# EmanueleCosenza/polyphemus

Hardware: AMD Instinct MI355X
Metric: bar-graphs/sec VAE fwd+bwd (+loss +Adam), LMD2 4-track x 32-ts synthetic (higher is better)
Workload: dtype f32 (fp16-pair MFMA products)

## Files before the change

include/polyphemus_hip.h:

```cpp
#ifndef POLYPHEMUS_HIP_H
#define POLYPHEMUS_HIP_H

#include <stdint.h>

#ifdef __cplusplus
extern "C" {
#endif

typedef void* pm_stream_t;

enum {
  PM_OK = 0,
  PM_E_INVALID = -1,
  PM_E_LAUNCH = -2,
  PM_E_UNSUPPORTED = -3
};

enum { PM_N_REL = 6, PM_N_DIST = 32, PM_N_SLOTS = 15, PM_N_PITCH = 131, PM_N_DUR = 99, PM_N_TOK = 230 };

#define PM_ABI_VERSION 9
int pm_abi_version(void);
const char* pm_build_info(void);

int pm_set_deterministic(int32_t on);
// ... 152 lines not shown
                               const float* bias , int32_t use_classes, float* h ,
                               double* col_stats , pm_stream_t stream);
int pm_gcl_forward_from_planes_h2(const uint16_t* a_planes, int64_t plane_stride, const int32_t* plan, int32_t N, int32_t E,
                                  int32_t G, int32_t d, const uint16_t* w_frag, const float* bias, int32_t use_classes,
                                  float* h, double* col_stats, const float* a_scale, float w_scale, pm_stream_t stream);
int pm_rows_times_weight(const float* X, int32_t ldx, int32_t N, int32_t K, const uint16_t* w_frag, int32_t kind,
                         int32_t w_tiles, int32_t Nout, const float* bias , float* C, int32_t ldc,
                         pm_stream_t stream);
int pm_rows_times_weight_longk(const float* X, int32_t ldx, int32_t N, int32_t K, const uint16_t* w_frag, int32_t kind,
                               int32_t w_pitch, int32_t Nout, float* C, int32_t ldc, pm_stream_t stream);
int pm_rows_tn_weight_grad(const float* A, int32_t lda, int32_t M, const float* B, int32_t ldb, int32_t Nn, int32_t K,
                           float* C , int32_t ldc, float* colsum_a , pm_stream_t stream);
typedef struct PmNormSums {
  const float* h;
  const float* mean; const float* var; const float* gamma; const float* beta;
  float eps; int32_t relu;
  double* acc3;
  uint32_t* absmax_out;
} PmNormSums;
int pm_segreduce_bwd_norm(const float* x, const float* T, const float* dA, const float* dres, const int32_t* plan,
                          int32_t N, int32_t E, int32_t G, int32_t d, float dropout_p, uint32_t seed,
                          uint32_t layer_uid, int32_t compact, float* dx, float* dT, const PmNormSums* next_norm,
                          pm_stream_t stream);
int pm_segreduce_bwd(const float* x, const float* T, const float* dA ,
                     const float* dres ,
                     const int32_t* plan, int32_t N, int32_t E, int32_t G, int32_t d, float dropout_p,
                     uint32_t seed, uint32_t layer_uid, int32_t compact, float* dx ,
                     float* dT , pm_stream_t stream);

int pm_bar_aggregate_fwd(const float* x, const float* T, const int32_t* plan, int32_t N, int32_t E, int32_t G, int32_t d,
                         float dropout_p, uint32_t seed, uint32_t layer_uid, uint16_t* planes, int64_t plane_stride,
                         const PmH2* h2 , pm_stream_t stream);
int pm_bar_aggregate_bwd(const float* x, const float* T, const float* dA , const float* dres ,
                         const int32_t* plan, int32_t N, int32_t E, int32_t G, int32_t d, float dropout_p, uint32_t seed,
                         uint32_t layer_uid, float* dx , float* dT ,
                         const PmNormSums* next_norm , pm_stream_t stream);

enum { PM_GEMM_RELU = 1, PM_GEMM_ACCUM = 2,
       PM_GEMM_RELU_ADD = 16 ,
       PM_GEMM_ZEROED = 8 ,
       PM_GEMM_PARTITION = 4  };
int pm_gemm_config(int32_t transA, int32_t M, int32_t N, int32_t K);
int pm_gemm_force_config(int32_t cfg);
int pm_gemm_f32(int transA, int transB, int32_t M, int32_t N, int32_t K, const float* A, int32_t lda,
                const float* B, int32_t ldb, float* C, int32_t ldc, const float* bias, int flags,
                int split_k, const int32_t* rowmap, int32_t rows_per_entry, const int32_t* dyn_entries,
// ... 110 lines not shown
int pm_embed_gather(const float* tables, const int32_t* tokens , const uint8_t* is_drum,
                    int32_t N, int32_t d, int32_t n_slots, float* X , pm_stream_t stream);
int pm_embed_bwd_scatter(const float* dX , const int32_t* tokens, const int32_t* plan, int32_t N,
                         int32_t E, int32_t G, int32_t d, int32_t n_slots,
                         float* S , pm_stream_t stream);
int pm_chord_pad_fwd(const float* tables, const float* chord_w , const float* chord_b,
                     const uint8_t* is_drum, int32_t N, int32_t d, int32_t n_slots, float* cvec ,
                     float* y , pm_stream_t stream);
int pm_chord_pad_bwd(const float* dy , const uint8_t* is_drum, int32_t N, int32_t d, int32_t n_slots,
                     const float* tables, const float* chord_w, float* gsum ,
                     float* d_chord_w , float* S , pm_stream_t stream);
int pm_chord_pad_vec(const float* tables, const float* chord_w, const float* chord_b, int32_t d, int32_t n_slots,
                     float* cvec , pm_stream_t stream);
int pm_chord_tables_fwd(const float* tables , const float* chord_w , int32_t d, int32_t n_slots,
                        float* PT, const float* chord_b , float* cvec ,
                        pm_stream_t stream);
int pm_chord_sum_fwd(const float* PT, const float* cvec, const int32_t* tokens , const uint8_t* is_drum, int32_t N,
                     int32_t d, int32_t n_slots, float* x0 , pm_stream_t stream);
int pm_chord_sum_bwd(const float* dy , const int32_t* tokens, const int32_t* plan, int32_t N, int32_t E, int32_t G,
                     int32_t d , int32_t n_slots, float* Gt, pm_stream_t stream);
int pm_chord_tables_bwd_w(const float* Gt, const float* tables, int32_t d, int32_t n_slots, float* d_chord_w ,
                          float* d_chord_b , pm_stream_t stream);
int pm_chord_tables_bwd_x(const float* Gt, const float* chord_w, int32_t d, int32_t n_slots, float* S , pm_stream_t stream);
int pm_embed_tables_bwd(const float* S, const float* w_pitch_drum, const float* b_pitch_drum,
                        const float* w_pitch_nd, const float* b_pitch_nd, const float* w_dur, const float* b_dur,
                        const float* bn_drum_g, const float* bn_nd_g, const float* bn_dur_g, const float* stats,
                        const int32_t* tok_hist, int32_t d, float eps, float* dw_pitch_drum, float* db_pitch_drum,
                        float* dw_pitch_nd, float* db_pitch_nd, float* dw_dur, float* db_dur, float* dg_drum,
                        float* dbeta_drum, float* dg_nd, float* dbeta_nd, float* dg_dur, float* dbeta_dur,
                        pm_stream_t stream);

int pm_embed_tables_bwd_sync(const float* S, const float* w_pitch_drum, const float* b_pitch_drum, const float* w_pitch_nd,
                             const float* b_pitch_nd, const float* w_dur, const float* b_dur, const float* bn_drum_g,
                             const float* bn_nd_g, const float* bn_dur_g, const float* stats, const int32_t* tok_hist,
                             int32_t d, float eps, float* dw_pitch_drum, float* db_pitch_drum, float* dw_pitch_nd,
                             float* db_pitch_nd, float* dw_dur, float* db_dur, float* dg_drum, float* dbeta_drum,
                             float* dg_nd, float* dbeta_nd, float* dg_dur, float* dbeta_dur, double* sums_out,
                             const double* sums_global, const int32_t* hist_global, pm_stream_t stream);

int pm_gate_fwd(const float* x , const float* w , const float* b , int32_t N,
                int32_t d, float* g , pm_stream_t stream);
int pm_attnpool_fwd(const float* x, const float* g, const float* g_mean, const float* g_var, float eps,
                    const float* bn_g, const float* bn_b, const int32_t* plan, int32_t N, int32_t E, int32_t G,
                    int32_t d, float* alpha , float* out , pm_stream_t stream);
int pm_attnpool_bwd(const float* x, const float* g, const float* g_mean, const float* g_var, float eps,
                    const float* bn_g, const float* alpha, const float* dout , const float* gate_w,
// ... 240 lines not shown
```

polyphemus_amd/_lib.py:

```python
from __future__ import annotations

import ctypes as C
import os
from typing import Optional

import torch

_HERE = os.path.dirname(os.path.abspath(__file__))
LIB_PATH = os.environ.get("PM_LIB_PATH") or os.path.join(_HERE, "libpolyphemus_hip.so")

PROF_NCLASS = 40
PLAN_FIELDS = ["rowptr", "csr_src", "csr_dist", "csr_eid", "colptr", "csc_dst", "csc_reldist", "csc_eid",
               "csc_invcnt", "node_bar", "bar_ptr", "group_list", "group_cnt", "tok_hist", "row_list", "node_trel", "trk_list", "trk_cnt", "scratch"]

_SIGS = {
    "pm_plan_layout": "iiip",
    "pm_gcl_tile_order": "piipi",
    "pm_row_tile_order": "ipi",
    "pm_plan_build": "pppppppiiiiips",
    "pm_edge_attrs_to_ids": "pipps",
    "pm_tokens_from_onehot": "pips",
    "pm_batch_flags": "pppiipps",
    "pm_edge_table": "ppips",
    "pm_edge_table_bwd": "pipps",
    "pm_graph_count": "pippppps",
    "pm_graph_emit": "piippllppppppps",
    "pm_binary_from_logits": "pifpps",
    "pm_mtp_from_logits": "ppilppps",
    "pm_segreduce_fwd": "pppiiiifuuips",
    "pm_segreduce_fwd_planes": "pppiiiifuuipls",
    "pm_gcl_forward_fused": "pppiiiifuuppipppls",
    "pm_gcl_input_grad_fused": "plpiiiipips",
    "pm_gcl_input_grad_bn": "pplpiiiipips",
    "pm_chord_pad_vec": "pppiips",
    "pm_chord_tables_fwd": "ppiippps",
    "pm_chord_sum_fwd": "ppppiiips",
    "pm_chord_sum_bwd": "pppiiiiips",
    "pm_chord_tables_bwd_w": "ppiipps",
    "pm_chord_tables_bwd_x": "ppiips",
    "pm_bn_bwd_sums": "ppiippfppips",
    "pm_gcl_weight_grad_fused": "plplpiiiiips",
    "pm_gcl_forward_from_planes": "plpiiiippipps",
    "pm_rows_times_weight": "piiipiiippis",
    "pm_rows_times_weight_longk": "piiipiiipis",
    "pm_rows_tn_weight_grad": "piipiiipips",
    "pm_segreduce_bwd": "pppppiiiifuuipps",
    "pm_segreduce_bwd_norm": "pppppiiiifuuippps",
    "pm_gemm_f32": "iiiiipipipipiipips",
    "pm_gemm_f32_grouped": "iiiiipipipipiipipilllliis",
    "pm_gemm_f32_desc": "ps",
    "pm_gemm_config": "iiii",
    "pm_gemm_force_config": "i",
    "pm_bn_stats": "piiippppfps",
    "pm_bn_small_fwd": "piifpppipppppfs",
    "pm_bn_small_bwd": "ppiippfppipppps",
    "pm_bn_apply": "piiippfpppips",
    "pm_bn_partial_sums": "ppiiippfppipps",
    "pm_bn_stats_from_sums": "pDippppfs",
    "pm_bn_bwd_from_sums": "ppiiippfppippDppppps",
    "pm_bn_bwd": "ppiiippfppippppps",
    "pm_bn_apply_fused": "piipfpppipppppfs",
    "pm_bn_bwd_fused": "ppiippfppipppppplis",
    "pm_split_planes": "plpls",
    "pm_split_planes_frag": "piiiillps",
    "pm_relu_bwd": "pplps",
    "pm_add": "pplps",
    "pm_bn_counters_update": "ppppis",
    "pm_grad_accumulate": "pplfis",
    "pm_colsum_acc": "piiips",
    "pm_colsum_rows_acc": "piipipips",
# ... 226 lines not shown
```

polyphemus_amd/csrc/chord.hip:

```cpp
#include "common.h"
#include <stdlib.h>

#define EMB_V PM_N_PITCH

namespace {
__host__ __device__ inline int64_t pt_off(int g, int s, int kind, int S, int d) {
  return (((int64_t)g * S + s) * 2 + kind) * EMB_V * d;
}

template <bool AK, bool BK, int KC, class FA, class FB, class FC>
__device__ inline void small_product(int M, int Nn, int K, int m0, int n0, FA a_at, FB b_at, FC c_out) {
  constexpr int PA = 34, PB = 68;
  constexpr int NA = KC / 8, NB = KC / 4;
  static_assert(KC % 8 == 0, "32 x KC and 64 x KC values over 256 threads");
  __shared__ __attribute__((aligned(16))) float sA[KC * PA], sB[KC * PB];
  const int t = threadIdx.x, tm = t >> 4, tn = t & 15;
  float acc[2][4] = {{0.f, 0.f, 0.f, 0.f}, {0.f, 0.f, 0.f, 0.f}};
  float ra[NA], rb[NB];
  auto request = [&](int k0) {
#pragma unroll
    for (int i = 0; i < NA; ++i) {
      const int idx = t + i * 256;
      const int m = AK ? idx / KC : idx & 31, k = AK ? idx % KC : idx >> 5;
      ra[i] = (m0 + m < M && k0 + k < K) ? a_at(m0 + m, k0 + k) : 0.f;
    }
#pragma unroll
    for (int i = 0; i < NB; ++i) {
      const int idx = t + i * 256;
      const int n = BK ? idx / KC : idx & 63, k = BK ? idx % KC : idx >> 6;
      rb[i] = (n0 + n < Nn && k0 + k < K) ? b_at(n0 + n, k0 + k) : 0.f;
    }
  };
  request(0);
  for (int k0 = 0; k0 < K; k0 += KC) {
#pragma unroll
    for (int i = 0; i < NA; ++i) {
      const int idx = t + i * 256;
      const int m = AK ? idx / KC : idx & 31, k = AK ? idx % KC : idx >> 5;
// ... 38 lines not shown
      const float* td = tables + ((int64_t)(2 + g) * EMB_V + 98) * dh;
      float a0 = 0.f, a1 = 0.f, a2 = 0.f, a3 = 0.f;
      const int i0 = S * d + lane, i1 = PM_N_SLOTS * d;
      int i = i0;
      for (; i + 192 < i1; i += 256) {
        const int c0 = i % d, c1 = (i + 64) % d, c2 = (i + 128) % d, c3 = (i + 192) % d;
        a0 += (c0 < dh ? tp[c0] : td[c0 - dh]) * wrow[i];
        a1 += (c1 < dh ? tp[c1] : td[c1 - dh]) * wrow[i + 64];
        a2 += (c2 < dh ? tp[c2] : td[c2 - dh]) * wrow[i + 128];
        a3 += (c3 < dh ? tp[c3] : td[c3 - dh]) * wrow[i + 192];
      }
      for (; i < i1; i += 64) { const int c0 = i % d; a0 += (c0 < dh ? tp[c0] : td[c0 - dh]) * wrow[i]; }
      const float acc = pm_wave_sum((a0 + a1) + (a2 + a3));
      if (lane == 0) cvec[g * d + o] = acc + bc[o];
    }
    return;
  }
  const int mt = blockIdx.x / ntn, nt = blockIdx.x % ntn, s = blockIdx.y, kind = blockIdx.z >> 1, g = blockIdx.z & 1;
  const int V = kind == 0 ? PM_N_PITCH : PM_N_DUR;
  if (mt * 32 >= V) return;
  const float* T = tables + (int64_t)(kind * 2 + g) * EMB_V * dh;
  const float* W = Wc + (int64_t)s * d + kind * dh;
  float* out = PT + pt_off(g, s, kind, S, d);
  small_product<true, true, 64>(V, d, dh, mt * 32, nt * 64,
                            [&](int v, int c) { return T[(int64_t)v * dh + c]; },
                            [&](int j, int c) { return W[(int64_t)j * PM_N_SLOTS * d + c]; },
                            [&](int v, int j, float x) { out[(int64_t)v * d + j] = x; });
}
extern "C" int pm_chord_tables_fwd(const float* tables, const float* Wc, int32_t d, int32_t n_slots, float* PT, const float* bc,
                                   float* cvec, pm_stream_t stream) {
  if (!tables || !Wc || !PT || d <= 0 || (d & 7) || n_slots < 1 || n_slots > PM_N_SLOTS || (cvec && !bc)) return PM_E_INVALID;
  const int ntm = (int)pm_cdiv(EMB_V, 32), ntn = (int)pm_cdiv(d, 64);
  hipLaunchKernelGGL(k_chord_tables_fwd, dim3(ntm * ntn, n_slots, cvec ? 5 : 4), dim3(256), 0, (hipStream_t)stream, tables, Wc, d,
                     n_slots, PT, bc, cvec);
  return pm_check_launch();
}

template <int SMAX>
__global__ void __launch_bounds__(256) k_chord_sum_fwd(const float* __restrict__ PT, const float* __restrict__ cvec,
                                                       const int* __restrict__ tok, const uint8_t* __restrict__ is_drum, int N,
                                                       int d, int S, float* __restrict__ x0, unsigned* __restrict__ absmax) {
  const int n = blockIdx.x * 4 + (threadIdx.x >> 6), lane = threadIdx.x & 63;
  __shared__ unsigned s_amax;
  if (threadIdx.x == 0) s_amax = 0u;
  float amax = 0.f;
  if (n < N) {
  const int g = is_drum[n] ? 0 : 1;
// ... 208 lines not shown
    Gv[(int64_t)pad * d + j] = all - oth;
  }
}
extern "C" int pm_chord_sum_bwd(const float* dY, const int32_t* tokens, const int32_t* plan, int32_t N, int32_t E, int32_t G_,
                                int32_t d, int32_t n_slots, float* Gt, pm_stream_t stream) {
  if (!dY || !tokens || !plan || !Gt || N <= 0 || d <= 0 || (d % 32) || d > 512 || n_slots < 1 || n_slots > PM_N_SLOTS ||
      (int64_t)N * d * 4 >= 0x7fffffffLL)
    return PM_E_INVALID;
  hipStream_t st = (hipStream_t)stream;
  PmPlanView pv = pm_plan_view(plan, N, E, G_);
  constexpr int chunk_env = 0;
  const int per = chunk_env > 0 ? chunk_env : 640;
  constexpr bool skip_pad = true;
  const int nb = (int)pm_cdiv(N, per) + 1;
  const int waves = d / 32 > 8 ? 8 : d / 32, cblks = (d / 32 + waves - 1) / waves;
  if (d / 32 != waves * cblks) return PM_E_INVALID;
  hipLaunchKernelGGL(k_chord_sum_bwd, dim3(nb, n_slots, 2 * cblks), dim3(64 * waves), 0, st, dY, tokens, pv.group_list, pv.group_cnt,
                     N, d, n_slots, per, skip_pad ? 1 : 0, Gt, pm_det_gate(st));
  if (skip_pad && 2 * n_slots > 1)
    hipLaunchKernelGGL(k_chord_pad_fix, dim3((unsigned)pm_cdiv(d, 64), 2 * n_slots, 2), dim3(256), 0, st, Gt, d, n_slots);
  return pm_check_launch();
}

__global__ void __launch_bounds__(256) k_chord_tables_bwd_w(const float* __restrict__ G, const float* __restrict__ tables, int d,
                                                            int S, float* __restrict__ dWc, float* __restrict__ db, unsigned* gate) {
  const int dh = d / 2, ntn = (dh + 63) / 64;
  const int mt = blockIdx.x / ntn, nt = blockIdx.x % ntn, s = blockIdx.y, kind = blockIdx.z >> 1, g = blockIdx.z & 1;
  const int V = kind == 0 ? PM_N_PITCH : PM_N_DUR;
  const float* Gg = G + pt_off(g, s, kind, S, d);
  const float* T = tables + (int64_t)(kind * 2 + g) * EMB_V * dh;
  float* out = dWc + (int64_t)s * d + kind * dh;
  float res[2][4];
  small_product<false, false, 72>(d, dh, V, mt * 32, nt * 64,
                                  [&](int j, int k) { return Gg[(int64_t)k * d + j]; },
                                  [&](int c, int k) { return T[(int64_t)k * dh + c]; },
                                  [&](int j, int c, float x) { res[(j - mt * 32) & 1][(c - nt * 64) & 3] = x; });
  float dbv = 0.f;
  const bool bias_part = db && s == 0 && kind == 0 && nt == 0;
  const int jb = mt * 32 + (threadIdx.x & 31);
  if (bias_part) {
    const int part = threadIdx.x >> 5;
    __shared__ float red[8][32];
    float a = 0.f;
    if (jb < d) {
      float v[17];
#pragma unroll
      for (int i = 0; i < 17; ++i) v[i] = part + 8 * i < V ? Gg[(int64_t)(part + 8 * i) * d + jb] : 0.f;
#pragma unroll
      for (int i = 0; i < 17; ++i) a += v[i];
    }
    red[part][threadIdx.x & 31] = a;
    __syncthreads();
    if (part == 0)
#pragma unroll
      for (int p = 0; p < 8; ++p) dbv += red[p][threadIdx.x & 31];
  }
  const int tm = threadIdx.x >> 4, tn = threadIdx.x & 15;
  pm_turn_enter_block(gate);
#pragma unroll
  for (int i = 0; i < 2; ++i)
#pragma unroll
    for (int j = 0; j < 4; ++j) {
      const int jj = mt * 32 + tm * 2 + i, c = nt * 64 + tn * 4 + j;
      if (jj < d && c < dh) atomicAdd(&out[(int64_t)jj * PM_N_SLOTS * d + c], res[i][j]);
    }
  if (bias_part && (threadIdx.x >> 5) == 0 && jb < d) atomicAdd(&db[jb], dbv);
  pm_turn_leave_block(gate);
}
__global__ void __launch_bounds__(256) k_chord_tables_bwd_x(const float* __restrict__ G, const float* __restrict__ Wc, int d, int S,
                                                            float* __restrict__ Stab, unsigned* gate) {
  const int dh = d / 2, ntn = (dh + 63) / 64;
  const int mt = blockIdx.x / ntn, nt = blockIdx.x % ntn, kind = blockIdx.y >> 1, g = blockIdx.y & 1, s = blockIdx.z >> 1;
  const int j0 = (blockIdx.z & 1) * dh;
  const int V = kind == 0 ? PM_N_PITCH : PM_N_DUR;
  if (mt * 32 >= V) { pm_turn_skip_block(gate); return; }
  const float* Gg = G + pt_off(g, s, kind, S, d) + j0;
  const float* W = Wc + (int64_t)j0 * PM_N_SLOTS * d + (int64_t)s * d + kind * dh;
  float* out = Stab + (int64_t)(kind * 2 + g) * EMB_V * dh;
  float res[2][4];
  small_product<true, false, 64>(V, dh, dh, mt * 32, nt * 64,
                                 [&](int v, int j) { return Gg[(int64_t)v * d + j]; },
                                 [&](int c, int j) { return W[(int64_t)j * PM_N_SLOTS * d + c]; },
                                 [&](int v, int c, float x) { res[(v - mt * 32) & 1][(c - nt * 64) & 3] = x; });
  const int tm = threadIdx.x >> 4, tn = threadIdx.x & 15;
  pm_turn_enter_block(gate);
#pragma unroll
  for (int i = 0; i < 2; ++i)
#pragma unroll
    for (int j = 0; j < 4; ++j) {
      const int v = mt * 32 + tm * 2 + i, c = nt * 64 + tn * 4 + j;
      if (v < V && c < dh) atomicAdd(&out[(int64_t)v * dh + c], res[i][j]);
    }
  pm_turn_leave_block(gate);
}
extern "C" int pm_chord_tables_bwd_w(const float* Gt, const float* tables, int32_t d, int32_t n_slots, float* dWc, float* db,
                                     pm_stream_t stream) {
  if (!Gt || !tables || !dWc || d <= 0 || (d & 7) || n_slots < 1 || n_slots > PM_N_SLOTS) return PM_E_INVALID;
  const int dh = d / 2;
  hipLaunchKernelGGL(k_chord_tables_bwd_w, dim3((unsigned)(pm_cdiv(d, 32) * pm_cdiv(dh, 64)), n_slots, 4), dim3(256), 0,
                     (hipStream_t)stream, Gt, tables, d, n_slots, dWc, db, pm_det_gate((hipStream_t)stream));
  return pm_check_launch();
}
extern "C" int pm_chord_tables_bwd_x(const float* Gt, const float* Wc, int32_t d, int32_t n_slots, float* Stab, pm_stream_t stream) {
  if (!Gt || !Wc || !Stab || d <= 0 || (d & 7) || n_slots < 1 || n_slots > PM_N_SLOTS) return PM_E_INVALID;
  hipStream_t st = (hipStream_t)stream;
  const int dh = d / 2;
  hipLaunchKernelGGL(k_chord_tables_bwd_x, dim3((unsigned)(pm_cdiv(EMB_V, 32) * pm_cdiv(dh, 64)), 4, 2 * n_slots), dim3(256), 0, st,
                     Gt, Wc, d, n_slots, Stab, pm_det_gate(st));
  return pm_check_launch();
}
```

polyphemus_amd/csrc/segreduce.hip:

```cpp
#include "common.h"
#include <string.h>
#include <stdlib.h>
#include "prof.h"

extern "C" uint32_t pm_dropout_hash(uint32_t seed, uint32_t layer_uid, uint32_t eid, uint32_t channel) {
  return pm_elem_hash(pm_edge_key(seed, layer_uid, eid), channel) >> 8;
}

__global__ void k_edge_table(const float* __restrict__ w, const float* __restrict__ b, int d, float* T) {
  const int i = blockIdx.x * blockDim.x + threadIdx.x;
  if (i >= PM_N_DIST * d) return;
  const int dist = i / d, c = i % d;
  T[i] = w[c * PM_N_DIST + dist] + b[c];
}
__global__ void k_edge_table_bwd(const float* __restrict__ dT, int d, float* dw, float* db) {
  const int c = blockIdx.x * blockDim.x + threadIdx.x;
  if (c >= d) return;
  float s = 0.f;
  for (int dist = 0; dist < PM_N_DIST; ++dist) {
    const float g = dT[dist * d + c];
    dw[c * PM_N_DIST + dist] += g;
    s += g;
  }
  db[c] += s;
// ... 125 lines not shown
extern "C" int pm_segreduce_fwd_planes(const float* x, const float* T, const int32_t* plan, int32_t N, int32_t E,
                                       int32_t G, int32_t d, float dropout_p, uint32_t seed, uint32_t layer_uid,
                                       int32_t compact, uint16_t* planes, int64_t plane_stride, pm_stream_t stream) {
  if (!planes) return PM_E_INVALID;
  return segreduce_fwd_impl(x, T, plan, N, E, G, d, dropout_p, seed, layer_uid, compact, nullptr, planes, plane_stride,
                            stream);
}

#ifndef SEG_KEEP
#define SEG_KEEP 1
#endif
#ifndef SEG_EPT
#define SEG_EPT 4
#endif
template <int NV, bool DROP, bool FUSE, bool RL>
__global__ void __launch_bounds__(1024) k_segreduce_bwd(const float* __restrict__ x, const float* __restrict__ T,
                                                       const float* __restrict__ dA, const float* __restrict__ dres,
                                                       const int* __restrict__ colptr, const int* __restrict__ csc_dst,
                                                       const int* __restrict__ csc_reldist,
                                                       const int* __restrict__ csc_eid,
                                                       const float* __restrict__ csc_invcnt, int N, int d,
                                                       uint32_t seed, uint32_t layer_uid, uint32_t thresh, float scale,
                                                       int compact, float* __restrict__ dx, float* __restrict__ dT,
                                                       PmNormSums nn, int xcd_nodes, int pr, unsigned* gate) {
  constexpr int EPT = NV == 1 ? SEG_EPT : 2;
  extern __shared__ __attribute__((aligned(16))) float sT[];
  const int nwv0 = blockDim.x >> 6;
  for (int i = threadIdx.x; i < (PM_N_DIST + nwv0 * pr) * d + 1; i += blockDim.x) sT[i] = 0.f;
  __syncthreads();
  const int lane = threadIdx.x & 63;
  const int wave = threadIdx.x >> 6;
  float* const sP = sT + PM_N_DIST * d + wave * pr * d;
  const int nblk = compact ? 4 : 7;
  const int dq = d >> 2;
  int c[NV];
  bool ok[NV];
#pragma unroll
  for (int v = 0; v < NV; ++v) { c[v] = (lane + v * 64) * 4; ok[v] = c[v] < d; }
  const int nwv = blockDim.x >> 6;
  constexpr bool KEEP = NV == 1 && SEG_KEEP;
  float nm[NV][4], nrs[NV][4], nga[NV][4], nbe[NV][4];
  double ns0[NV][4], ns1[NV][4], ns2[NV][4];
  if (FUSE) {
#pragma unroll
    for (int v = 0; v < NV; ++v)
#pragma unroll
      for (int j = 0; j < 4; ++j) {
// ... 114 lines not shown
          }
          if (RL) {
            if (dist[u] != prev[u]) flush_run(v, prev[u]);
#pragma unroll
            for (int j = 0; j < 4; ++j) run[v][j] += gt[j];
          } else {
#pragma unroll
            for (int j = 0; j < 4; ++j) run[v][j] = gt[j];
            flush_run(v, dist[u]);
          }
        }
      }
      cur = dist[EPT - 1];
    }
    if (RL) {
#pragma unroll
      for (int v = 0; v < NV; ++v)
        if (ok[v]) flush_run(v, cur);
    }
    cur = -1;
#pragma unroll
    for (int v = 0; v < NV; ++v) {
      if (!ok[v]) continue;
      *reinterpret_cast<float4*>(dx + (int64_t)n * d + c[v]) = acc[v];
      if (FUSE) {
        if constexpr (NV == 1)
          amax = fmaxf(fmaxf(amax, fmaxf(fabsf(acc[v].x), fabsf(acc[v].y))), fmaxf(fabsf(acc[v].z), fabsf(acc[v].w)));
        const float4 hv = *reinterpret_cast<const float4*>(nn.h + (int64_t)n * d + c[v]);
        const float hs[4] = {hv.x, hv.y, hv.z, hv.w};
        const float ds[4] = {acc[v].x, acc[v].y, acc[v].z, acc[v].w};
        float m4[4], r4[4], g4n[4], b4[4];
        if (KEEP) {
#pragma unroll
          for (int j = 0; j < 4; ++j) { m4[j] = nm[v][j]; r4[j] = nrs[v][j]; g4n[j] = nga[v][j]; b4[j] = nbe[v][j]; }
        } else {
          const float4 mv = *reinterpret_cast<const float4*>(nn.mean + c[v]), vv = *reinterpret_cast<const float4*>(nn.var + c[v]);
          const float4 gv = *reinterpret_cast<const float4*>(nn.gamma + c[v]), bv = *reinterpret_cast<const float4*>(nn.beta + c[v]);
          m4[0] = mv.x; m4[1] = mv.y; m4[2] = mv.z; m4[3] = mv.w;
          r4[0] = rsqrtf(vv.x + nn.eps); r4[1] = rsqrtf(vv.y + nn.eps); r4[2] = rsqrtf(vv.z + nn.eps); r4[3] = rsqrtf(vv.w + nn.eps);
          g4n[0] = gv.x; g4n[1] = gv.y; g4n[2] = gv.z; g4n[3] = gv.w;
          b4[0] = bv.x; b4[1] = bv.y; b4[2] = bv.z; b4[3] = bv.w;
        }
#pragma unroll
        for (int j = 0; j < 4; ++j) {
          const float xh = (hs[j] - m4[j]) * r4[j];
          float du = ds[j];
          if (nn.relu && !(xh * g4n[j] + b4[j] > 0.f)) du = 0.f;
// ... 53 lines not shown
      double t = 0;
      for (int q = 0; q < nslot; ++q) t += sd[(int64_t)q * 3 * d + i];
      atomicAdd(&dst[i], t);
    }
  }
  pm_turn_leave_block(gate);
}

template <int NV, bool DR, bool FU, bool RL>
static void seg_bwd_lds_attr(size_t lds) {
  static size_t granted_dev[16] = {};
  size_t& granted = granted_dev[pm_device_slot()];
  if (granted == 0) granted = 64 * 1024;
  if (lds > granted) {
    hipFuncSetAttribute(reinterpret_cast<const void*>(&k_segreduce_bwd<NV, DR, FU, RL>),
                        hipFuncAttributeMaxDynamicSharedMemorySize, (int)lds);
    granted = lds;
  }
}

static int segreduce_bwd_impl(const float* x, const float* T, const float* dA, const float* dres, const int32_t* plan,
                              int32_t N, int32_t E, int32_t G, int32_t d, float dropout_p, uint32_t seed,
                              uint32_t layer_uid, int32_t compact, float* dx, float* dT, const PmNormSums* nn,
                              pm_stream_t stream) {
  if (!x || !T || !dA || !plan || !dx || !dT || N <= 0 || d <= 0 || (d & 3) || d > 1024 || dropout_p < 0.f ||
      dropout_p >= 1.f)
    return PM_E_INVALID;
  if (nn && (!nn->h || !nn->mean || !nn->var || !nn->gamma || !nn->beta || !nn->acc3)) return PM_E_INVALID;
  PmPlanView pv = pm_plan_view(plan, N, E, G);
  hipStream_t st = (hipStream_t)stream;
  unsigned* const gate = pm_det_gate(st);
  constexpr int dev_waves = 0;
  constexpr int dev_blocks = 0;
  const int threads = gate ? 64 : (N >= 4096 ? (dev_waves > 0 && dev_waves <= 16 ? dev_waves * 64 : 1024) : 256);
  int nblk = (int)pm_cdiv(N, threads / 64);
  const int cap = gate ? 512 : (dev_blocks > 0 ? dev_blocks : 256);
  if (nblk > cap) nblk = cap;
  const dim3 grid(nblk), block(threads);
  int xcd_nodes = 0;
  if (seg_xcd_aware() && nblk >= 16 && (nblk & 7) == 0) xcd_nodes = (int)pm_cdiv(pm_cdiv(N, 8), threads / 64) * (threads / 64);
  constexpr int pr_cap = 4;
  int pr = (int)((144 * 1024 / sizeof(float) / d - PM_N_DIST) / (threads / 64));
  if (pr > pr_cap) pr = pr_cap;
  if (pr < 0) pr = 0;
  const size_t lds = sizeof(float) * ((PM_N_DIST + (size_t)(threads / 64) * pr) * d + 4);
  const bool drop = dropout_p > 0.f;
  const uint32_t thresh = pm_keep_threshold(dropout_p);
  const float scale = drop ? 1.0f / (1.0f - dropout_p) : 1.0f;
  PmNormSums none;
  memset(&none, 0, sizeof(none));
  const PmNormSums nv_ = nn ? *nn : none;
#define LAUNCH(NV, DR, FU, RL)                                                                                       \
  do { seg_bwd_lds_attr<NV, DR, FU, RL>(lds);                                                                     \
  hipLaunchKernelGGL((k_segreduce_bwd<NV, DR, FU, RL>), grid, block, lds, st, x, T, dA, dres, pv.colptr, pv.csc_dst,  \
                     pv.csc_reldist, pv.csc_eid, pv.csc_invcnt, N, d, seed, layer_uid, thresh, scale, compact, dx, dT, nv_, xcd_nodes, pr, gate); } while (0)
  const bool rl = d <= 256 || (int64_t)E >= 16 * (int64_t)N;
#define LAUNCH2(NV, DR) do { if (nn) { if (rl) LAUNCH(NV, DR, true, true); else LAUNCH(NV, DR, true, false); }       \
                             else { if (rl) LAUNCH(NV, DR, false, true); else LAUNCH(NV, DR, false, false); } } while (0)
  const int nv = (int)pm_cdiv(d, 256);
  const int pe = pm_prof_open(st, PM_PROF_SEGREDUCE_BWD, 4.0 * d * (double)N * ((compact ? 4 : PM_N_REL + 1) + 1 + (dres ? 1 : 0) + (nn ? 1 : 0)) + 12.0 * E + 128.0 * d);
  if (nv == 1) { if (drop) LAUNCH2(1, true); else LAUNCH2(1, false); }
  else if (nv == 2) { if (drop) LAUNCH2(2, true); else LAUNCH2(2, false); }
  else { if (drop) LAUNCH2(4, true); else LAUNCH2(4, false); }
#undef LAUNCH2
#undef LAUNCH
  pm_prof_close(st, pe);
  return pm_check_launch();
}
extern "C" int pm_segreduce_bwd(const float* x, const float* T, const float* dA, const float* dres, const int32_t* plan,
                                int32_t N, int32_t E, int32_t G, int32_t d, float dropout_p, uint32_t seed,
                                uint32_t layer_uid, int32_t compact, float* dx, float* dT, pm_stream_t stream) {
  return segreduce_bwd_impl(x, T, dA, dres, plan, N, E, G, d, dropout_p, seed, layer_uid, compact, dx, dT, nullptr, stream);
}
extern "C" int pm_segreduce_bwd_norm(const float* x, const float* T, const float* dA, const float* dres,
                                     const int32_t* plan, int32_t N, int32_t E, int32_t G, int32_t d, float dropout_p,
                                     uint32_t seed, uint32_t layer_uid, int32_t compact, float* dx, float* dT,
                                     const PmNormSums* next_norm, pm_stream_t stream) {
  if (!next_norm) return PM_E_INVALID;
  return segreduce_bwd_impl(x, T, dA, dres, plan, N, E, G, d, dropout_p, seed, layer_uid, compact, dx, dT, next_norm, stream);
}
```

polyphemus_amd/csrc/vae_step.hip:

```cpp
#include "common.h"
#include <stdio.h>
#include <string.h>
#include <mutex>

int pm_plan_build_marked(const int64_t* edge_index, const int32_t* edge_type, const int32_t* edge_dist, const int64_t* bars,
                         const int64_t* batch, const uint8_t* is_drum, const int32_t* tokens, int32_t n_bars, int32_t n_slots,
                         int32_t N, int32_t E, int32_t G, int32_t* plan, hipStream_t stream, hipEvent_t after_count);
extern "C" int pm_kld_acc(const float* mu, const float* log_var, int32_t B, int32_t d, float beta, float* dmu, float* dlog_var,
                          double* out, pm_stream_t stream);
extern "C" int pm_chord_sum_fwd_absmax(const float* PT, const float* cvec, const int32_t* tokens, const uint8_t* is_drum, int32_t N, int32_t d,
                                       int32_t n_slots, float* x0, uint32_t* absmax, pm_stream_t stream);
extern "C" int pm_bn_bwd_sums_absmax(const float* x, const float* dy, int32_t O, int32_t C, const float* mean, const float* var, float eps,
                                     const float* gamma, const float* beta, int relu, double* acc3, uint32_t* absmax_dy,
                                     pm_stream_t stream);
extern "C" int pm_bce_logits_acc(const float* logits, const float* target, int64_t n, float grad_scale, float* dlogits, double* out,
                                 pm_stream_t stream);
namespace {

struct StepCfg {
  bool gcl_fused, no_dw, no_rows_w, no_classes, fused_ce, debug;
  int side_stream;
  int side_delay_us;
  bool dagg_bn;
  bool dagg_res;
  bool chord_tables;
  bool plan_side;
  bool h2;
  bool senc_first;
  bool unembed_dw;
  bool pad_skip;
  bool cnn_fused;
  bool bar_route;
  int64_t offset_limit;
};
static StepCfg read_cfg() {
  auto flag = [](const char* n, bool dflt) { const char* v = getenv(n); return v ? atoi(v) != 0 : dflt; };
  StepCfg k;
  k.gcl_fused = flag("PM_GCL_FUSED", true);
  k.no_dw = flag("PM_GCL_NO_DW", false);
  k.no_rows_w = flag("PM_NO_ROWS_W", false);
  k.no_classes = getenv("PM_GCL_NO_CLASSES") != nullptr;
  k.fused_ce = flag("PM_FUSED_CE", true);
  k.debug = getenv("PM_DEBUG") != nullptr;
  k.side_stream = getenv("PM_SIDE_STREAM") ? atoi(getenv("PM_SIDE_STREAM")) : 0xffff;
  k.dagg_bn = flag("PM_DAGG_BN", true);
  k.plan_side = flag("PM_PLAN_SIDE", true);
  k.chord_tables = flag("PM_CHORD_TABLES", true);
  k.dagg_res = flag("PM_DAGG_RES", true);
  k.h2 = flag("PM_H2", true);
  k.side_delay_us = getenv("PM_SIDE_DELAY_US") ? atoi(getenv("PM_SIDE_DELAY_US")) : 0;
  k.bar_route = flag("PM_BAR_ROUTE", true);
  k.pad_skip = flag("PM_PAD_SKIP", true);
  k.unembed_dw = flag("PM_UNEMBED_DW", true);
  k.senc_first = flag("PM_SENC_FIRST", true);
  k.cnn_fused = flag("PM_CNN_FUSED", true);
  k.offset_limit = getenv("PM_GCL_OFFSET_LIMIT") ? atoll(getenv("PM_GCL_OFFSET_LIMIT")) : 0x7fffffffLL;
  return k;
}
static StepCfg g_cfg = read_cfg();
static const StepCfg& cfg() { return g_cfg; }

struct Arena {
  char* base; size_t cap, used; bool overflow;
  size_t zcap, zused;
  void* take(size_t bytes) {
    const size_t a = (used + 255) & ~size_t(255);
    used = a + bytes;
    if (!base) return nullptr;
    if (zcap + used > cap) { overflow = true; return base + zcap; }
    return base + zcap + a;
  }
  void* z(size_t bytes) {
    const size_t a = (zused + 255) & ~size_t(255);
    zused = a + bytes;
    if (!base) return nullptr;
    if (zused > zcap) { overflow = true; return base; }
    return base + a;
  }
// ... 422 lines not shown
        q.M = N; q.N = d; q.K = 4 * d;
        q.A = sv.A[i]; q.lda = 4 * d; q.B = W; q.ldb = d; q.C = sv.h[i]; q.ldc = d; q.bias = bias;
        q.b_group_stride = dd; q.b_split_rows = d; q.b_shared_off = 3 * dd;
        q.col_stats = sums;
        if (c.planes) {
          q.operand_planes = 1; q.A = (const float*)sv.Ap[i]; q.a_plane_stride = aps;
          q.B = (const float*)(sv.Wp + (g.weight[i] - sv.wp_base)); q.b_plane_stride = sv.wp_stride;
          q.b_frag = Wf;
        }
        RUN(pm_gemm_f32_desc(&q, c.st));
        break;
      }
    }
    const PmBn& bn = g.norm[i];
    if (c.bn)
      RUN(pm_bn_apply_fused_absmax(sv.h[i], N, d, sums, 1e-5f, c.P + bn.w, c.P + bn.b, sv.x[i], 1, sv.x[i + 1], sv.mean[i],
                                     sv.var[i], c.Bf + bn.rm, c.Bf + bn.rv, 0.1f,
                                     (r.x_tracked && i + 1 < c.L) ? sv.mx + (i + 1) * PM_ABSMAX_SLOTS : nullptr, c.st));
    else
      RUN(pm_relu_residual_fwd(sv.h[i], sv.x[i], (int64_t)N * d, sv.x[i + 1], c.st));
  }
  return sv.x[c.L];
}
float* gcn_backward(Ctx& c, float* dx, const PmGcn& g, GcnSaved& sv) {
  Arena& ar = c.s->ar;
  const int N = c.N, d = c.d, nb = c.compact ? 4 : 7;
  const int64_t dd = (int64_t)d * d;
  float* dT = ar.zf((size_t)PM_N_DIST * d);
  float* dh = ar.f((size_t)N * d);
  float* dA = ar.f((size_t)N * nb * d);
  const int64_t aps = (int64_t)N * nb * d, dps = (int64_t)N * d;
  uint16_t* const dhp = c.planes ? (uint16_t*)ar.take((size_t)dps * 6) : nullptr;
  float* dxa = ar.f((size_t)N * d);
  float* dxb = ar.f((size_t)N * d);
  PmPlanView pv = pm_plan_view(c.s->plan, N, c.E, c.Gn);
  float* dxin = c.pdrop > 0.f ? ar.f((size_t)N * d) : nullptr;
  const GcnRoute& r = sv.rt;
  for (int i = c.L - 1; i >= 0; --i) {
    const float* W = c.P + g.weight[i];
    float* dW = c.G + g.weight[i];
    const PmBn& bn = g.norm[i];
    const uint16_t* Wf = r.frag ? sv.Wft + (int64_t)i * sv.wf_stride : nullptr;
    double* const acc3 = sv.pool + ((size_t)i * 5 + 2) * d * PM_BN_REPL;
    const bool sums_ready = i < c.L - 1 && r.bagg_sums;
    const bool du_tracked = sums_ready && r.bagg_absmax, du_from_sums = r.norm == GcnRoute::NORM_IN_DAGG && !sums_ready;
    PmH2 h2 = {};
    if (r.h2) { h2.absmax_in = sv.mdu + i * PM_ABSMAX_SLOTS; h2.scale_out = sv.sdh + i; h2.w_scale = kH2WScale; }
// ... 79 lines not shown
    PmNormSums nn;
    const bool carry = i > 0 && r.bagg_sums;
    if (carry) {
      const PmBn& pb = g.norm[i - 1];
      nn.h = sv.h[i - 1]; nn.mean = sv.mean[i - 1]; nn.var = sv.var[i - 1]; nn.gamma = c.P + pb.w; nn.beta = c.P + pb.b;
      nn.eps = 1e-5f; nn.relu = 1; nn.acc3 = sv.pool + ((size_t)(i - 1) * 5 + 2) * d * PM_BN_REPL;
      nn.absmax_out = r.bagg_absmax ? sv.mdu + (i - 1) * PM_ABSMAX_SLOTS : nullptr;
    }
    switch (r.bagg) {
      case GcnRoute::BAGG_SEG_DROPPED:
        RUN(pm_segreduce_bwd(sv.xin[i], sv.T, dA, nullptr, c.s->plan, N, c.E, c.Gn, d, sv.p, sv.seed, sv.uid0 + i, c.compact, dxin,
                               dT, c.st));
        drop(c, dxin, N, d, sv.site0 + i, sv.seed, dxin);
        RUN(pm_add(dx, dxin, (int64_t)N * d, out, c.st));
        break;
      case GcnRoute::BAGG_BAR:
        RUN(pm_bar_aggregate_bwd(sv.x[i], sv.T, dA, res, c.s->plan, N, c.E, c.Gn, d, sv.p, sv.seed, sv.uid0 + i, out, dT,
                                   carry ? &nn : nullptr, c.st));
        break;
      case GcnRoute::BAGG_SEG:
        if (carry)
          RUN(pm_segreduce_bwd_norm(sv.x[i], sv.T, dA, res, c.s->plan, N, c.E, c.Gn, d, sv.p, sv.seed, sv.uid0 + i, c.compact, out,
                                      dT, &nn, c.st));
        else
          RUN(pm_segreduce_bwd(sv.x[i], sv.T, dA, res, c.s->plan, N, c.E, c.Gn, d, sv.p, sv.seed, sv.uid0 + i, c.compact, out, dT, c.st));
        break;
    }
    dx = out;
  }
  RUN(pm_edge_table_bwd(dT, d, c.G + g.nn_w, c.G + g.nn_b, c.st));
  return dx;
}

Ctx make_ctx(StepState* s, hipStream_t st) {
  Ctx c;
  c.s = s; c.st = st; c.rc = PM_OK; c.bn_scratch = s->bn_scratch;
  c.N = s->bt.N; c.E = s->bt.E; c.Gn = s->bt.G; c.B = s->bt.B;
  c.d = s->lay.d; c.nb = s->lay.n_bars; c.L = s->lay.n_layers;
  c.S = s->bt.n_slots;
  c.compact = (s->bt.flags & 1) ? 1 : 0;
  c.planes = (c.compact && (s->bt.flags & 2) && (s->lay.d % 8) == 0) ? 1 : 0;
  c.P = s->P; c.G = s->G; c.Bf = s->Bf;
  c.bn = !(s->lay.flags & 1); c.pdrop = s->lay.dropout;
  return c;
}


// ... 477 lines not shown
  }
  float* dxL = ar.f((size_t)N * d);
  float* pscr = ar.f((size_t)3 * N + 8);
  const bool dropping = c.pdrop > 0.f;
  float* dxg = dropping ? ar.f((size_t)N * d) : nullptr;
  RUN(pm_attnpool_bwd(s.eg.x[c.L], s.g, s.gm, s.gv, 1e-5f, c.P + Y.enc_gate_bn.w, s.alpha, dpooled, c.P + Y.enc_gate.w,
                        s.plan, N, c.E, Gn, d, dxL, c.G + Y.enc_gate.w, c.G + Y.enc_gate.b, c.G + Y.enc_gate_bn.w,
                        c.G + Y.enc_gate_bn.b, pscr, dropping ? s.xLg : nullptr, dxg, c.st));
  if (dropping) {
    drop(c, dxg, N, d, SITE_ENC_GATE, s.seed_enc, dxg);
    RUN(pm_add(dxL, dxg, (int64_t)N * d, dxL, c.st));
  }
  branch_join(c, BR_DEC_WGRAD);
  s.bk_dxL = dxL; s.bk_dzcat = dzcat;
}
void backward_encoder(Ctx& c) {
  StepState& s = *c.s;
  const PmVaeLayout& Y = s.lay;
  const int N = c.N, d = c.d;
  if (!s.bk_dxL) backward_encoder_heads(c);
  float* dxL = s.bk_dxL;
  float* dzcat = s.bk_dzcat;
  s.bk_dxL = nullptr;
  float* dx0 = gcn_backward(c, dxL, Y.enc_gcn, s.eg);
  drop(c, dx0, N, d, SITE_ENC_CHORD, s.seed_enc, dx0);
  RUN(pm_relu_bwd(dx0, s.x0, (int64_t)N * d, dx0, c.st));
  branch_join(c, BR_ENC_HEAD_WGRAD);
  s.bk_dx0 = dx0; s.bk_dzcat = dzcat;
}
void backward_encoder_tail(Ctx& c) {
  StepState& s = *c.s;
  Arena& ar = s.ar;
  const PmVaeLayout& Y = s.lay;
  const int N = c.N, Gn = c.Gn, B = c.B, d = c.d, nb = c.nb, dh = d / 2;
  float* dx0 = s.bk_dx0;
  float* dzcat = s.bk_dzcat;
  const int S = c.S;
  const HeadRoute& rt = s.head;
  const bool chord_tab = chord_tab_ok(c);
  float* dX = chord_tab ? nullptr : ar.f((size_t)N * S * d);
  float* Stab = chord_tab ? ar.zf((size_t)4 * PM_N_PITCH * dh) : ar.f((size_t)4 * PM_N_PITCH * dh);
  float* gsum = ar.f((size_t)2 * d);
  float* Gt = chord_tab ? ar.zf((size_t)2 * S * 2 * PM_N_PITCH * d) : nullptr;
  if (rt.chord == HeadRoute::CHORD_TABLES) {
    {
      BranchScope br(c, BR_ENC_WGRAD);
      RUN(pm_chord_pad_bwd(dx0, s.bt.is_drum, N, d, S, s.tables, c.P + Y.enc_chord.w, gsum, c.G + Y.enc_chord.w, Stab, c.st));
      br.pause();
      RUN(pm_chord_sum_bwd(dx0, s.bt.tokens, s.plan, N, c.E, Gn, d, S, Gt, c.st));
      br.wait_main();
      br.resume();
      RUN(pm_chord_tables_bwd_x(Gt, c.P + Y.enc_chord.w, d, S, Stab, c.st));
      br.pause();
      RUN(pm_chord_tables_bwd_w(Gt, s.tables, d, S, c.G + Y.enc_chord.w, c.G + Y.enc_chord.b, c.st));
    }
    branch_join(c, BR_ENC_WGRAD);
  } else if (rt.chord == HeadRoute::CHORD_FULL) lin_bwd(c, dx0, s.X, Y.enc_chord, N, d, PM_N_SLOTS * d, dX);
  else {
    {
      BranchScope br(c, BR_ENC_WGRAD);
      if (rt.chord_dw_tn)
        RUN(pm_rows_tn_weight_grad(dx0, d, d, s.X, S * d, S * d, N, c.G + Y.enc_chord.w, PM_N_SLOTS * d, c.G + Y.enc_chord.b, c.st));
      else {
        PmGemmDesc w;
        memset(&w, 0, sizeof(w));
        w.transA = 1; w.M = d; w.N = S * d; w.K = N; w.A = dx0; w.lda = d; w.B = s.X; w.ldb = S * d;
        w.C = c.G + Y.enc_chord.w; w.ldc = PM_N_SLOTS * d; w.flags = PM_GEMM_ACCUM; w.split_k = 0; w.n_groups = 1;
        w.a_colsum = c.G + Y.enc_chord.b;
// ... 261 lines not shown
```

Measured before the change: 137,100.

## Fuse chord-table weight and input grads into one launch; fold ReLU into segreduce bwd

New measurement: 137,600, median of 6. About the same (+0.4%).

```diff
diff --git a/include/polyphemus_hip.h b/include/polyphemus_hip.h
--- a/include/polyphemus_hip.h
+++ b/include/polyphemus_hip.h
@@ -198,6 +198,10 @@
                           int32_t N, int32_t E, int32_t G, int32_t d, float dropout_p, uint32_t seed,
                           uint32_t layer_uid, int32_t compact, float* dx, float* dT, const PmNormSums* next_norm,
                           pm_stream_t stream);
+int pm_segreduce_bwd_relu(const float* x, const float* T, const float* dA, const float* dres, const int32_t* plan,
+                          int32_t N, int32_t E, int32_t G, int32_t d, float dropout_p, uint32_t seed,
+                          uint32_t layer_uid, int32_t compact, float* dx, float* dT, const PmNormSums* next_norm ,
+                          pm_stream_t stream);
 int pm_segreduce_bwd(const float* x, const float* T, const float* dA ,
                      const float* dres ,
                      const int32_t* plan, int32_t N, int32_t E, int32_t G, int32_t d, float dropout_p,
@@ -354,6 +358,8 @@
 int pm_chord_tables_bwd_w(const float* Gt, const float* tables, int32_t d, int32_t n_slots, float* d_chord_w ,
                           float* d_chord_b , pm_stream_t stream);
 int pm_chord_tables_bwd_x(const float* Gt, const float* chord_w, int32_t d, int32_t n_slots, float* S , pm_stream_t stream);
+int pm_chord_tables_bwd_wx(const float* Gt, const float* tables, const float* chord_w, int32_t d, int32_t n_slots,
+                           float* d_chord_w , float* d_chord_b , float* S , pm_stream_t stream);
 int pm_embed_tables_bwd(const float* S, const float* w_pitch_drum, const float* b_pitch_drum,
                         const float* w_pitch_nd, const float* b_pitch_nd, const float* w_dur, const float* b_dur,
                         const float* bn_drum_g, const float* bn_nd_g, const float* bn_dur_g, const float* stats,
diff --git a/polyphemus_amd/_lib.py b/polyphemus_amd/_lib.py
--- a/polyphemus_amd/_lib.py
+++ b/polyphemus_amd/_lib.py
@@ -38,6 +38,7 @@
     "pm_chord_sum_bwd": "pppiiiiips",
     "pm_chord_tables_bwd_w": "ppiipps",
     "pm_chord_tables_bwd_x": "ppiips",
+    "pm_chord_tables_bwd_wx": "pppiippps",
     "pm_bn_bwd_sums": "ppiippfppips",
     "pm_gcl_weight_grad_fused": "plplpiiiiips",
     "pm_gcl_forward_from_planes": "plpiiiippipps",
@@ -46,6 +47,7 @@
     "pm_rows_tn_weight_grad": "piipiiipips",
     "pm_segreduce_bwd": "pppppiiiifuuipps",
     "pm_segreduce_bwd_norm": "pppppiiiifuuippps",
+    "pm_segreduce_bwd_relu": "pppppiiiifuuippps",
     "pm_gemm_f32": "iiiiipipipipiipips",
     "pm_gemm_f32_grouped": "iiiiipipipipiipipilllliis",
     "pm_gemm_f32_desc": "ps",
diff --git a/polyphemus_amd/csrc/chord.hip b/polyphemus_amd/csrc/chord.hip
--- a/polyphemus_amd/csrc/chord.hip
+++ b/polyphemus_amd/csrc/chord.hip
@@ -8,12 +8,12 @@
   return (((int64_t)g * S + s) * 2 + kind) * EMB_V * d;
 }
 
+constexpr int SP_PA = 34, SP_PB = 68;
 template <bool AK, bool BK, int KC, class FA, class FB, class FC>
-__device__ inline void small_product(int M, int Nn, int K, int m0, int n0, FA a_at, FB b_at, FC c_out) {
-  constexpr int PA = 34, PB = 68;
+__device__ inline void small_product(float* sA, float* sB, int M, int Nn, int K, int m0, int n0, FA a_at, FB b_at, FC c_out) {
+  constexpr int PA = SP_PA, PB = SP_PB;
   constexpr int NA = KC / 8, NB = KC / 4;
   static_assert(KC % 8 == 0, "32 x KC and 64 x KC values over 256 threads");
-  __shared__ __attribute__((aligned(16))) float sA[KC * PA], sB[KC * PB];
   const int t = threadIdx.x, tm = t >> 4, tn = t & 15;
   float acc[2][4] = {{0.f, 0.f, 0.f, 0.f}, {0.f, 0.f, 0.f, 0.f}};
   float ra[NA], rb[NB];
@@ -98,7 +98,8 @@
   const float* T = tables + (int64_t)(kind * 2 + g) * EMB_V * dh;
   const float* W = Wc + (int64_t)s * d + kind * dh;
   float* out = PT + pt_off(g, s, kind, S, d);
-  small_product<true, true, 64>(V, d, dh, mt * 32, nt * 64,
+  __shared__ __attribute__((aligned(16))) float sA[64 * SP_PA], sB[64 * SP_PB];
+  small_product<true, true, 64>(sA, sB, V, d, dh, mt * 32, nt * 64,
                             [&](int v, int c) { return T[(int64_t)v * dh + c]; },
                             [&](int j, int c) { return W[(int64_t)j * PM_N_SLOTS * d + c]; },
                             [&](int v, int j, float x) { out[(int64_t)v * d + j] = x; });
@@ -353,16 +354,17 @@
   return pm_check_launch();
 }
 
-__global__ void __launch_bounds__(256) k_chord_tables_bwd_w(const float* __restrict__ G, const float* __restrict__ tables, int d,
-                                                            int S, float* __restrict__ dWc, float* __restrict__ db, unsigned* gate) {
+__device__ inline void chord_tables_bwd_w_body(int bx, int by, int bz, float* sA, float* sB, const float* __restrict__ G,
+                                               const float* __restrict__ tables, int d, int S, float* __restrict__ dWc,
+                                               float* __restrict__ db, unsigned* gate) {
   const int dh = d / 2, ntn = (dh + 63) / 64;
-  const int mt = blockIdx.x / ntn, nt = blockIdx.x % ntn, s = blockIdx.y, kind = blockIdx.z >> 1, g = blockIdx.z & 1;
+  const int mt = bx / ntn, nt = bx % ntn, s = by, kind = bz >> 1, g = bz & 1;
   const int V = kind == 0 ? PM_N_PITCH : PM_N_DUR;
   const float* Gg = G + pt_off(g, s, kind, S, d);
   const float* T = tables + (int64_t)(kind * 2 + g) * EMB_V * dh;
   float* out = dWc + (int64_t)s * d + kind * dh;
   float res[2][4];
-  small_product<false, false, 72>(d, dh, V, mt * 32, nt * 64,
+  small_product<false, false, 72>(sA, sB, d, dh, V, mt * 32, nt * 64,
                                   [&](int j, int k) { return Gg[(int64_t)k * d + j]; },
                                   [&](int c, int k) { return T[(int64_t)k * dh + c]; },
                                   [&](int j, int c, float x) { res[(j - mt * 32) & 1][(c - nt * 64) & 3] = x; });
@@ -398,18 +400,23 @@
   if (bias_part && (threadIdx.x >> 5) == 0 && jb < d) atomicAdd(&db[jb], dbv);
   pm_turn_leave_block(gate);
 }
-__global__ void __launch_bounds__(256) k_chord_tables_bwd_x(const float* __restrict__ G, const float* __restrict__ Wc, int d, int S,
-                                                            float* __restrict__ Stab, unsigned* gate) {
+__global__ void __launch_bounds__(256) k_chord_tables_bwd_w(const float* __restrict__ G, const float* __restrict__ tables, int d,
+                                                            int S, float* __restrict__ dWc, float* __restrict__ db, unsigned* gate) {
+  __shared__ __attribute__((aligned(16))) float sA[72 * SP_PA], sB[72 * SP_PB];
+  chord_tables_bwd_w_body(blockIdx.x, blockIdx.y, blockIdx.z, sA, sB, G, tables, d, S, dWc, db, gate);
+}
+__device__ inline void chord_tables_bwd_x_body(int bx, int by, int bz, float* sA, float* sB, const float* __restrict__ G,
+                                               const float* __restrict__ Wc, int d, int S, float* __restrict__ Stab, unsigned* gate) {
   const int dh = d / 2, ntn = (dh + 63) / 64;
-  const int mt = blockIdx.x / ntn, nt = blockIdx.x % ntn, kind = blockIdx.y >> 1, g = blockIdx.y & 1, s = blockIdx.z >> 1;
-  const int j0 = (blockIdx.z & 1) * dh;
+  const int mt = bx / ntn, nt = bx % ntn, kind = by >> 1, g = by & 1, s = bz >> 1;
+  const int j0 = (bz & 1) * dh;
   const int V = kind == 0 ? PM_N_PITCH : PM_N_DUR;
   if (mt * 32 >= V) { pm_turn_skip_block(gate); return; }
   const float* Gg = G + pt_off(g, s, kind, S, d) + j0;
   const float* W = Wc + (int64_t)j0 * PM_N_SLOTS * d + (int64_t)s * d + kind * dh;
   float* out = Stab + (int64_t)(kind * 2 + g) * EMB_V * dh;
   float res[2][4];
-  small_product<true, false, 64>(V, dh, dh, mt * 32, nt * 64,
+  small_product<true, false, 64>(sA, sB, V, dh, dh, mt * 32, nt * 64,
                                  [&](int v, int j) { return Gg[(int64_t)v * d + j]; },
                                  [&](int c, int j) { return W[(int64_t)j * PM_N_SLOTS * d + c]; },
                                  [&](int v, int c, float x) { res[(v - mt * 32) & 1][(c - nt * 64) & 3] = x; });
@@ -423,6 +430,19 @@
       if (v < V && c < dh) atomicAdd(&out[(int64_t)v * dh + c], res[i][j]);
     }
   pm_turn_leave_block(gate);
+}
+__global__ void __launch_bounds__(256) k_chord_tables_bwd_x(const float* __restrict__ G, const float* __restrict__ Wc, int d, int S,
+                                                            float* __restrict__ Stab, unsigned* gate) {
+  __shared__ __attribute__((aligned(16))) float sA[64 * SP_PA], sB[64 * SP_PB];
+  chord_tables_bwd_x_body(blockIdx.x, blockIdx.y, blockIdx.z, sA, sB, G, Wc, d, S, Stab, gate);
+}
+__global__ void __launch_bounds__(256) k_chord_tables_bwd_wx(const float* __restrict__ G, const float* __restrict__ tables,
+                                                             const float* __restrict__ Wc, int d, int S, float* __restrict__ dWc,
+                                                             float* __restrict__ db, float* __restrict__ Stab, int nx, int xg0, int wg0) {
+  __shared__ __attribute__((aligned(16))) float sA[72 * SP_PA], sB[72 * SP_PB];
+  const int b = blockIdx.x;
+  if (b < nx) chord_tables_bwd_x_body(b % xg0, (b / xg0) & 3, b / (xg0 * 4), sA, sB, G, Wc, d, S, Stab, nullptr);
+  else { const int w = b - nx; chord_tables_bwd_w_body(w % wg0, (w / wg0) % S, w / (wg0 * S), sA, sB, G, tables, d, S, dWc, db, nullptr); }
 }
 extern "C" int pm_chord_tables_bwd_w(const float* Gt, const float* tables, int32_t d, int32_t n_slots, float* dWc, float* db,
                                      pm_stream_t stream) {
@@ -440,3 +460,18 @@
                      Gt, Wc, d, n_slots, Stab, pm_det_gate(st));
   return pm_check_launch();
 }
+extern "C" int pm_chord_tables_bwd_wx(const float* Gt, const float* tables, const float* Wc, int32_t d, int32_t n_slots, float* dWc,
+                                      float* db, float* Stab, pm_stream_t stream) {
+  if (!Gt || !tables || !Wc || !dWc || !Stab || d <= 0 || (d & 7) || n_slots < 1 || n_slots > PM_N_SLOTS) return PM_E_INVALID;
+  hipStream_t st = (hipStream_t)stream;
+  if (pm_det_on()) {
+    const int rc = pm_chord_tables_bwd_w(Gt, tables, d, n_slots, dWc, db, stream);
+    return rc != PM_OK ? rc : pm_chord_tables_bwd_x(Gt, Wc, d, n_slots, Stab, stream);
+  }
+  const int dh = d / 2;
+  const int xg0 = (int)(pm_cdiv(EMB_V, 32) * pm_cdiv(dh, 64)), wg0 = (int)(pm_cdiv(d, 32) * pm_cdiv(dh, 64));
+  const int nx = xg0 * 4 * 2 * n_slots, nw = wg0 * n_slots * 4;
+  hipLaunchKernelGGL(k_chord_tables_bwd_wx, dim3((unsigned)(nx + nw)), dim3(256), 0, st, Gt, tables, Wc, d, n_slots, dWc, db, Stab, nx,
+                     xg0, wg0);
+  return pm_check_launch();
+}
diff --git a/polyphemus_amd/csrc/segreduce.hip b/polyphemus_amd/csrc/segreduce.hip
--- a/polyphemus_amd/csrc/segreduce.hip
+++ b/polyphemus_amd/csrc/segreduce.hip
@@ -171,7 +171,7 @@
                                                        const float* __restrict__ csc_invcnt, int N, int d,
                                                        uint32_t seed, uint32_t layer_uid, uint32_t thresh, float scale,
                                                        int compact, float* __restrict__ dx, float* __restrict__ dT,
-                                                       PmNormSums nn, int xcd_nodes, int pr, unsigned* gate) {
+                                                       PmNormSums nn, int xcd_nodes, int pr, unsigned* gate, int relu_x) {
   constexpr int EPT = NV == 1 ? SEG_EPT : 2;
   extern __shared__ __attribute__((aligned(16))) float sT[];
   const int nwv0 = blockDim.x >> 6;
@@ -332,7 +332,11 @@
 #pragma unroll
     for (int v = 0; v < NV; ++v) {
       if (!ok[v]) continue;
-      *reinterpret_cast<float4*>(dx + (int64_t)n * d + c[v]) = acc[v];
+      if (relu_x)
+        *reinterpret_cast<float4*>(dx + (int64_t)n * d + c[v]) = make_float4(xv[v].x > 0.f ? acc[v].x : 0.f, xv[v].y > 0.f ? acc[v].y : 0.f,
+                                                                             xv[v].z > 0.f ? acc[v].z : 0.f, xv[v].w > 0.f ? acc[v].w : 0.f);
+      else
+        *reinterpret_cast<float4*>(dx + (int64_t)n * d + c[v]) = acc[v];
       if (FUSE) {
         if constexpr (NV == 1)
           amax = fmaxf(fmaxf(amax, fmaxf(fabsf(acc[v].x), fabsf(acc[v].y))), fmaxf(fabsf(acc[v].z), fabsf(acc[v].w)));
@@ -432,7 +436,7 @@
 static int segreduce_bwd_impl(const float* x, const float* T, const float* dA, const float* dres, const int32_t* plan,
                               int32_t N, int32_t E, int32_t G, int32_t d, float dropout_p, uint32_t seed,
                               uint32_t layer_uid, int32_t compact, float* dx, float* dT, const PmNormSums* nn,
-                              pm_stream_t stream) {
+                              pm_stream_t stream, int relu_x = 0) {
   if (!x || !T || !dA || !plan || !dx || !dT || N <= 0 || d <= 0 || (d & 3) || d > 1024 || dropout_p < 0.f ||
       dropout_p >= 1.f)
     return PM_E_INVALID;
@@ -463,7 +467,7 @@
 #define LAUNCH(NV, DR, FU, RL)                                                                                       \
   do { seg_bwd_lds_attr<NV, DR, FU, RL>(lds);                                                                     \
   hipLaunchKernelGGL((k_segreduce_bwd<NV, DR, FU, RL>), grid, block, lds, st, x, T, dA, dres, pv.colptr, pv.csc_dst,  \
-                     pv.csc_reldist, pv.csc_eid, pv.csc_invcnt, N, d, seed, layer_uid, thresh, scale, compact, dx, dT, nv_, xcd_nodes, pr, gate); } while (0)
+                     pv.csc_reldist, pv.csc_eid, pv.csc_invcnt, N, d, seed, layer_uid, thresh, scale, compact, dx, dT, nv_, xcd_nodes, pr, gate, relu_x); } while (0)
   const bool rl = d <= 256 || (int64_t)E >= 16 * (int64_t)N;
 #define LAUNCH2(NV, DR) do { if (nn) { if (rl) LAUNCH(NV, DR, true, true); else LAUNCH(NV, DR, true, false); }       \
                              else { if (rl) LAUNCH(NV, DR, false, true); else LAUNCH(NV, DR, false, false); } } while (0)
@@ -489,3 +493,8 @@
   if (!next_norm) return PM_E_INVALID;
   return segreduce_bwd_impl(x, T, dA, dres, plan, N, E, G, d, dropout_p, seed, layer_uid, compact, dx, dT, next_norm, stream);
 }
+extern "C" int pm_segreduce_bwd_relu(const float* x, const float* T, const float* dA, const float* dres, const int32_t* plan,
+                                     int32_t N, int32_t E, int32_t G, int32_t d, float dropout_p, uint32_t seed, uint32_t layer_uid,
+                                     int32_t compact, float* dx, float* dT, const PmNormSums* next_norm, pm_stream_t stream) {
+  return segreduce_bwd_impl(x, T, dA, dres, plan, N, E, G, d, dropout_p, seed, layer_uid, compact, dx, dT, next_norm, stream, 1);
+}
diff --git a/polyphemus_amd/csrc/vae_step.hip b/polyphemus_amd/csrc/vae_step.hip
--- a/polyphemus_amd/csrc/vae_step.hip
+++ b/polyphemus_amd/csrc/vae_step.hip
@@ -30,6 +30,7 @@
   bool unembed_dw;
   bool pad_skip;
   bool cnn_fused;
+  bool chord_tail;
   bool bar_route;
   int64_t offset_limit;
 };
@@ -54,6 +55,7 @@
   k.unembed_dw = flag("PM_UNEMBED_DW", true);
   k.senc_first = flag("PM_SENC_FIRST", true);
   k.cnn_fused = flag("PM_CNN_FUSED", true);
+  k.chord_tail = flag("PM_CHORD_TAIL", true);
   k.offset_limit = getenv("PM_GCL_OFFSET_LIMIT") ? atoll(getenv("PM_GCL_OFFSET_LIMIT")) : 0x7fffffffLL;
   return k;
 }
@@ -522,7 +524,7 @@
   }
   return sv.x[c.L];
 }
-float* gcn_backward(Ctx& c, float* dx, const PmGcn& g, GcnSaved& sv) {
+float* gcn_backward(Ctx& c, float* dx, const PmGcn& g, GcnSaved& sv, const float* relu_x0 = nullptr, bool* relu_x0_done = nullptr) {
   Arena& ar = c.s->ar;
   const int N = c.N, d = c.d, nb = c.compact ? 4 : 7;
   const int64_t dd = (int64_t)d * d;
@@ -648,7 +650,11 @@
         if (carry)
           RUN(pm_segreduce_bwd_norm(sv.x[i], sv.T, dA, res, c.s->plan, N, c.E, c.Gn, d, sv.p, sv.seed, sv.uid0 + i, c.compact, out,
                                       dT, &nn, c.st));
-        else
+        else if (i == 0 && relu_x0 && relu_x0 == sv.x[0]) {
+          RUN(pm_segreduce_bwd_relu(sv.x[0], sv.T, dA, res, c.s->plan, N, c.E, c.Gn, d, sv.p, sv.seed, sv.uid0, c.compact, out, dT, nullptr,
+                                      c.st));
+          *relu_x0_done = true;
+        } else
           RUN(pm_segreduce_bwd(sv.x[i], sv.T, dA, res, c.s->plan, N, c.E, c.Gn, d, sv.p, sv.seed, sv.uid0 + i, c.compact, out, dT, c.st));
         break;
     }
@@ -1172,9 +1178,10 @@
   float* dxL = s.bk_dxL;
   float* dzcat = s.bk_dzcat;
   s.bk_dxL = nullptr;
-  float* dx0 = gcn_backward(c, dxL, Y.enc_gcn, s.eg);
+  bool relu_done = false;
+  float* dx0 = gcn_backward(c, dxL, Y.enc_gcn, s.eg, cfg().chord_tail && s.eg.x[0] == s.x0 ? s.x0 : nullptr, &relu_done);
   drop(c, dx0, N, d, SITE_ENC_CHORD, s.seed_enc, dx0);
-  RUN(pm_relu_bwd(dx0, s.x0, (int64_t)N * d, dx0, c.st));
+  if (!relu_done) RUN(pm_relu_bwd(dx0, s.x0, (int64_t)N * d, dx0, c.st));
   branch_join(c, BR_ENC_HEAD_WGRAD);
   s.bk_dx0 = dx0; s.bk_dzcat = dzcat;
 }
@@ -1193,7 +1200,14 @@
   float* gsum = ar.f((size_t)2 * d);
   float* Gt = chord_tab ? ar.zf((size_t)2 * S * 2 * PM_N_PITCH * d) : nullptr;
   if (rt.chord == HeadRoute::CHORD_TABLES) {
-    {
+    if (cfg().chord_tail) {
+      {
+        BranchScope br(c, BR_ENC_WGRAD);
+        RUN(pm_chord_pad_bwd(dx0, s.bt.is_drum, N, d, S, s.tables, c.P + Y.enc_chord.w, gsum, c.G + Y.enc_chord.w, Stab, c.st));
+      }
+      RUN(pm_chord_sum_bwd(dx0, s.bt.tokens, s.plan, N, c.E, Gn, d, S, Gt, c.st));
+      RUN(pm_chord_tables_bwd_wx(Gt, s.tables, c.P + Y.enc_chord.w, d, S, c.G + Y.enc_chord.w, c.G + Y.enc_chord.b, Stab, c.st));
+    } else {
       BranchScope br(c, BR_ENC_WGRAD);
       RUN(pm_chord_pad_bwd(dx0, s.bt.is_drum, N, d, S, s.tables, c.P + Y.enc_chord.w, gsum, c.G + Y.enc_chord.w, Stab, c.st));
       br.pause();
```
